# dominikh/jello

Hardware: AMD Instinct MI355X
Metric: Mpixels/sec fine-raster + paths/sec, 100k-path 4096^2 scene (higher is better)
Workload: dtype f32

## Files before the change

### jello_amd/csrc/kernels_flatten.hip

```cpp
#include <hip/hip_runtime.h>
__shared__ double fl_atan_tab[9];
#define JD_ATAN_TAB_LDS fl_atan_tab
#include "kcommon.h"
#define FF_INLINE __device__ __forceinline__
#include "flatten_fast.h"

using namespace jk;
using namespace jd;

namespace {

struct CubicParams { float th0, th1, chord_len, err; };
struct EulerParams { float th0, th1, k0, k1, ch; };
struct CubicPoints { V2 p0, p1, p2, p3; };
struct PointDeriv { V2 point, deriv; };
struct PathTagData { uint32_t tag_byte; MonoidK<5> monoid; };

#define DERIV_THRESH 1e-6f
#define DERIV_THRESH_SQUARED (DERIV_THRESH * DERIV_THRESH)
#define DERIV_EPS 1e-6f
#define SUBDIV_LIMIT (1.0f / 65536.0f)
#define K1_THRESH 1e-3f
#define DIST_THRESH 1e-3f
#define TANGENT_THRESH 1e-6f
// ... 725 lines not shown
            MonoidK<5> tot5;
            if (SCAN == 1) __syncthreads();
            const MonoidK<5> ex = block_excl_scan_monoid<5>(reduce_tag(tag_word), sh, &tot5);
            pm = monoid_add(prefix, ex);
            if (tag_monoids.ok(word_ix)) {
                store_tm(&tag_monoids.p[word_ix], pm);
            } else {
#pragma unroll
                for (int i = 0; i < 5; i++) pm.v[i] = 0u;
            }
            __syncthreads();
        } else {
            pm = load_tm(tag_monoids, word_ix);
        }
        const uint32_t ix0 = word_ix * 4u;
        for (uint32_t q = 0u; q < 12u; q++) {
            const uint32_t sl = ix0 * 3u + q;
            if (sl < cap) counts[sl] = 0u;
        }
        uint32_t th = 0u, tl = 0u;
#pragma unroll
        for (uint32_t k = 0; k < 4u; k++) {
            const uint32_t ix = ix0 + k;
            if (ix >= n_tags) continue;
            const MonoidK<5> tm = monoid_add(pm, reduce_tag(tag_word & ((1u << (k * 8u)) - 1u)));
            const uint32_t tag_byte = (tag_word >> (k * 8u)) & 0xffu;
            const uint32_t style_flags = scene.rd(cfg->layout.style_base + tm.v[3] - 2u);
            const bool is_stroke = (style_flags & JL_STYLE_FLAGS_STYLE) != 0u;
            const uint32_t path_ix = tm.v[4];
            if ((tag_byte & JL_PATH_TAG_PATH) != 0u && path_bboxes.ok(path_ix)) {
                path_bboxes.p[path_ix].draw_flags = ((style_flags & JL_STYLE_FLAGS_FILL) == 0u) ? 0u : 1u;
                path_bboxes.p[path_ix].trans_ix = tm.v[0] - 1u;
            }
            const uint32_t seg_type = tag_byte & JL_PATH_TAG_SEG_TYPE;
            const bool curved = seg_type != JL_PATH_TAG_LINETO;
            if (seg_type != 0u) {
                if (!is_stroke) {
                    if (curved) nh[blk][k] = 1u; else nl[blk][k] = 1u;
                } else if ((tag_byte & JL_PATH_TAG_SUBPATH_END) != 0u) {
                    if (curved) nl[blk][k] = 1u;
                } else {
                    if (curved) { nh[blk][k] = 2u; nl[blk][k] = 1u; } else { nl[blk][k] = 3u; }
                }
            }
            th += nh[blk][k];
            tl += nl[blk][k];
        }
        MonoidK<2> m, tot;
        m.v[0] = th; m.v[1] = tl;
        const MonoidK<2> e2 = block_excl_scan_monoid<2>(m, sh, &tot);
        eh[blk] = wg_h + e2.v[0];
        el[blk] = wg_l + e2.v[1];
        wg_h += tot.v[0];
        wg_l += tot.v[1];
        __syncthreads();
    }
    if (threadIdx.x == 0) {
        sh_base[0] = wg_h ? atomicAdd(&counters[0], wg_h) : 0u;
        sh_base[1] = wg_l ? atomicAdd(&counters[FL_CTR_LIGHT], wg_l) : 0u;
    }
    __syncthreads();
#pragma unroll
    for (uint32_t blk = 0; blk < PSC_BLOCKS; blk++) {
        const uint32_t ix0 = ((blockIdx.x * PSC_BLOCKS + blk) * JL_WG + threadIdx.x) * 4u;
        uint32_t ph = sh_base[0] + eh[blk], pl = sh_base[1] + el[blk];
#pragma unroll
        for (uint32_t k = 0; k < 4u; k++) {
            const uint32_t ix = ix0 + k;
            uint32_t sub = 0u;
            for (uint32_t q = 0; q < nh[blk][k]; q++, sub++, ph++)
                if (ph < cap) list[ph] = ix * 3u + sub;
            for (uint32_t q = 0; q < nl[blk][k]; q++, sub++, pl++)
                if (pl < cap) list[cap - 1u - pl] = ix * 3u + sub;
        }
    }
}

JD void run_item(const JlConfig* cfg, const Scene& s, Out& o, uint32_t slot, EulerJob& job, uint32_t& path_ix_out) {
    uint32_t ix = slot / 3u, sub = slot - ix * 3u;
    Seg g = load_seg(s, ix);
    uint32_t path_ix = g.tag.monoid.v[4];
    path_ix_out = path_ix;
    uint32_t style_ix = g.tag.monoid.v[3];
    uint32_t trans_ix = g.tag.monoid.v[0];
    uint32_t style_flags = g.style_flags;
    job.path_ix = path_ix; job.trans_ix = trans_ix;
    Xf transform;
    {
        uint32_t base = cfg->layout.transform_base + trans_ix * 6u;
        transform.m0 = u2f(s.scene.rd(base)); transform.m1 = u2f(s.scene.rd(base + 1u)); transform.m2 = u2f(s.scene.rd(base + 2u));
        transform.m3 = u2f(s.scene.rd(base + 3u)); transform.t0 = u2f(s.scene.rd(base + 4u)); transform.t1 = u2f(s.scene.rd(base + 5u));
    }
    CubicPoints pts = read_path_segment(s, g.tag, g.is_stroke);
    if (g.is_stroke) {
        float linewidth = u2f(s.scene.rd(cfg->layout.style_base + style_ix + 1u));
        float offset = 0.5f * linewidth;
        bool is_stroke_cap_marker = (g.tag.tag_byte & JL_PATH_TAG_SUBPATH_END) != 0u;
        if (is_stroke_cap_marker) {
            V2 tangent = cubic_start_tangent(pts.p0, pts.p1, pts.p2, pts.p3);
            V2 offset_tangent = offset * normalize(tangent);
            V2 n = v2(offset_tangent.y * -1.0f, offset_tangent.x * 1.0f);
            draw_cap(o, path_ix, (style_flags & JL_STYLE_FLAGS_START_CAP_MASK) >> 2, pts.p0, pts.p0 - n, pts.p0 + n, -offset_tangent, transform);
        } else {
            const float TT = TANGENT_THRESH * TANGENT_THRESH;
            V2 tan_prev = cubic_end_tangent(pts.p0, pts.p1, pts.p2, pts.p3);
            if (dot(tan_prev, tan_prev) < TT) tan_prev = v2(TANGENT_THRESH, 0.0f);
            V2 offset_tangent = offset * normalize(tan_prev);
            V2 n_prev = v2(offset_tangent.y * -1.0f, offset_tangent.x * 1.0f);
            if (sub < 2u) {
                V2 tan_start = cubic_start_tangent(pts.p0, pts.p1, pts.p2, pts.p3);
                if (dot(tan_start, tan_start) < TT) tan_start = v2(TANGENT_THRESH, 0.0f);
                V2 n_start = offset * normalize(v2(-tan_start.y, tan_start.x));
                job.valid = true; job.cubic = pts; job.local_to_device = transform;
                if (sub == 0u) { job.offset = offset; job.start_p = pts.p0 + n_start; job.end_p = pts.p3 + n_prev; }
                else { job.offset = -offset; job.start_p = pts.p0 - n_start; job.end_p = pts.p3 - n_prev; }
            } else {
                PathTagData ntag = compute_tag_monoid(s, ix + 1u);
                CubicPoints npts = read_path_segment(s, ntag, true);
                bool n_is_closed = (ntag.tag_byte & JL_PATH_TAG_SEG_TYPE) == JL_PATH_TAG_LINETO;
                bool n_is_marker = (ntag.tag_byte & JL_PATH_TAG_SUBPATH_END) != 0u;
                bool do_join = !n_is_marker || n_is_closed;
                if (do_join) {
                    V2 tan_next = cubic_start_tangent(npts.p0, npts.p1, npts.p2, npts.p3);
                    if (dot(tan_next, tan_next) < TT) tan_next = v2(TANGENT_THRESH, 0.0f);
                    V2 tnn = normalize(tan_next);
                    V2 n_next = v2((offset * tnn.y) * -1.0f, (offset * tnn.x) * 1.0f);
                    draw_join(o, path_ix, style_flags, pts.p3, tan_prev, tan_next, n_prev, n_next, transform);
                } else {
                    draw_cap(o, path_ix, (style_flags & JL_STYLE_FLAGS_END_CAP_MASK), pts.p3, pts.p3 + n_prev, pts.p3 - n_prev, offset_tangent, transform);
                }
            }
        }
    } else {
        job.valid = true; job.cubic = pts; job.local_to_device = transform;
        job.offset = 0.0f; job.start_p = pts.p0; job.end_p = pts.p3;
    }
}

#ifndef FLQ_STACK
#define FLQ_STACK 448u
#endif
#ifndef FLQ_LEAVES
#define FLQ_LEAVES 640u
#endif
#ifndef FLQ_MAX_LEVEL
#define FLQ_MAX_LEVEL 9u
#endif
struct FlBatch {
    uint32_t jhead[64];
    uint32_t stack[FLQ_STACK];
    uint32_t l_tpos[FLQ_LEAVES];
    uint16_t l_key[FLQ_LEAVES];
    uint16_t l_link[FLQ_LEAVES];
    uint32_t unsure[128];
    uint32_t n_stack, n_leaves, bail, n_unsure;
};

struct NodeResult {
    bool accept;
    CubicParams cp;
};
struct NodeEnds {
    V2 last_p, last_q;
    float last_t;
    V2 point, deriv;
    float t1;
};
JD NodeEnds node_ends(V2 p0, V2 p1, V2 p2, V2 p3, uint32_t level, uint32_t t0_u) {
    const float dt = u2f((127u - level) << 23);
    const float t0 = (float)t0_u * dt;
    NodeEnds r;
    if (t0_u == 0u) {
        r.last_p = p0;
        r.last_q = start_deriv(p0, p1, p2, p3);
        r.last_t = 0.0f;
    } else {
        PointDeriv pq0 = eval_cubic_and_deriv(p0, p1, p2, p3, t0);
        r.last_t = t0;
        if (dot(pq0.deriv, pq0.deriv) < DERIV_THRESH_SQUARED) {
            PointDeriv n0 = eval_cubic_and_deriv(p0, p1, p2, p3, t0 - DERIV_EPS);
            pq0.deriv = n0.deriv;
            pq0.point = n0.point;
            r.last_t = t0 - DERIV_EPS;
        }
        r.last_p = pq0.point;
        r.last_q = pq0.deriv;
    }
    const IntervalEnd ie = interval_end(p0, p1, p2, p3, t0 + dt);
    r.point = ie.pq.point;
    r.deriv = ie.pq.deriv;
    r.t1 = ie.t1;
    return r;
}
JD NodeResult node_test(V2 p0, V2 p1, V2 p2, V2 p3, float scale, uint32_t level, uint32_t t0_u) {
    const float tol = 0.25f;
    const float dt = u2f((127u - level) << 23);
    const NodeEnds ne = node_ends(p0, p1, p2, p3, level, t0_u);
    const float actual_dt = ne.t1 - ne.last_t;
    NodeResult r;
    r.cp = cubic_from_points_derivs(ne.last_p, ne.point, ne.last_q, ne.deriv, actual_dt);
    r.accept = r.cp.err * scale <= tol || dt <= SUBDIV_LIMIT;
    return r;
}
JD int node_test_fast(V2 p0, V2 p1, V2 p2, V2 p3, float scale, uint32_t level, uint32_t t0_u, float* v_est, float* delta) {
    const float tol = 0.25f;
    const NodeEnds ne = node_ends(p0, p1, p2, p3, level, t0_u);
    const float actual_dt = ne.t1 - ne.last_t;
    const V2 chord = ne.point - ne.last_p;
    const V2 q0 = ne.last_q, q1 = ne.deriv;
    *v_est = 0.0f; *delta = 0.0f;
    if (dot(chord, chord) < DERIV_THRESH_SQUARED) {
        const float chord_err = sqrt_((float)(9.0 / 32.0) * (dot(q0, q0) + dot(q1, q1))) * actual_dt;
        return (chord_err * scale <= tol) ? ffast::FF_ACCEPT : ffast::FF_REJECT;
    }
    return ffast::ff_decide_interval(chord.x, chord.y, q0.x, q0.y, q1.x, q1.y, actual_dt, scale, tol, v_est, delta);
}
JD CubicParams piece_angles(const NodeEnds& ne) {
    const V2 chord = ne.point - ne.last_p;
    const float chord_squared = dot(chord, chord);
    CubicParams r;
    r.err = 0.0f;
    if (chord_squared < DERIV_THRESH_SQUARED) {
        r.th0 = 0.0f; r.th1 = 0.0f; r.chord_len = DERIV_THRESH;
        return r;
    }
    const V2 q0 = ne.last_q, q1 = ne.deriv;
    const V2 h0 = v2(q0.x * chord.x + q0.y * chord.y, q0.y * chord.x - q0.x * chord.y);
    const V2 h1 = v2(q1.x * chord.x + q1.y * chord.y, q1.x * chord.y - q1.y * chord.x);
    r.th0 = atan2_(h0.y, h0.x);
    r.th1 = atan2_(h1.y, h1.x);
    r.chord_len = sqrt_(chord_squared);
    return r;
}


struct JobState { V2 p0, p1, p2, p3; float scale, offset; uint32_t slot, path_ix, trans_ix; V2 t_start, t_end; };
#define FL_JOB_CURVE(JB, E, J)                                                                                                      \
    JobState JB;                                                                                                                    \
    JB.p0 = v2(read_lane_var(E.p0.x, J), read_lane_var(E.p0.y, J)); JB.p1 = v2(read_lane_var(E.p1.x, J), read_lane_var(E.p1.y, J)); \
    JB.p2 = v2(read_lane_var(E.p2.x, J), read_lane_var(E.p2.y, J)); JB.p3 = v2(read_lane_var(E.p3.x, J), read_lane_var(E.p3.y, J)); \
    JB.scale = read_lane_var(E.scale, J)
#define FL_JOB_PIECE(JB, E, SLOT, J)                                                                                                \
    FL_JOB_CURVE(JB, E, J); JB.offset = read_lane_var(E.offset, J);                                                                 \
    JB.slot = read_lane_var(SLOT, J); JB.path_ix = read_lane_var(E.path_ix, J); JB.trans_ix = read_lane_var(E.trans_ix, J);         \
    JB.t_start = v2(read_lane_var(E.t_start.x, J), read_lane_var(E.t_start.y, J));                                                  \
    JB.t_end = v2(read_lane_var(E.t_end.x, J), read_lane_var(E.t_end.y, J))

#ifdef FL_FAST_CHECK
__device__ uint32_t g_ff_stats[8];
#endif
#ifndef FL_WAVES_PER_EU
#define FL_WAVES_PER_EU 4
#endif
#ifndef FL_BLOCKS_PER_CU
#define FL_BLOCKS_PER_CU 4
#endif
#ifdef FL_TIMING
#define FL_TL_WAVES 8192u
#define FL_TL_BATCHES 15u
#define FL_TL_WORDS (2u + 3u * FL_TL_BATCHES)
__device__ unsigned long long g_fl_timeline[FL_TL_WAVES * FL_TL_WORDS];
#endif
__global__ __launch_bounds__(JL_WG) __attribute__((amdgpu_waves_per_eu(FL_WAVES_PER_EU, FL_WAVES_PER_EU))) void k_flatten_items(const JlConfig* __restrict__ cfg, Buf<uint32_t> scene, Buf<JlTagMonoid> tag_monoids,
                                                         Buf<JlPathBbox> path_bboxes, const uint32_t* __restrict__ list,
                                                         uint32_t* __restrict__ counters, uint32_t cap, uint32_t* __restrict__ counts,
                                                         FlTemp T, uint32_t debug) {
    __shared__ FlBatch sh_batch[JL_WG / 64];
    Scene s;
    s.cfg = cfg; s.scene = scene; s.tag_monoids = tag_monoids;
    uint32_t n_heavy = umin_(counters[0], cap), n_light = umin_(counters[FL_CTR_LIGHT], cap - n_heavy);
    uint32_t n = n_heavy + n_light;
    const uint32_t units_h = n_heavy / 64u + (n_heavy % 64u != 0u ? 1u : 0u);
    const uint32_t units = units_h + n_light / 64u + (n_light % 64u != 0u ? 1u : 0u);
    const uint32_t n_groups = umin_(umax_(gridDim.x / FL_BLOCKS_PER_CU, 1u), FL_DEAL_GROUPS), group = blockIdx.x % n_groups;
    if (group >= units) return;
#ifdef FL_TIMING
    const unsigned long long tl_entry = wall_clock64();
    const uint32_t tl_wave = blockIdx.x * (JL_WG / 64u) + (threadIdx.x >> 6);
    uint32_t tl_n = 0u;
#endif
    atan_tab_fill();
    __syncthreads();
    const uint32_t lane = lane_id();
    FlBatch& B = sh_batch[threadIdx.x >> 6];
    Out o;
    o.cfg = cfg; o.T = T; o.home_s = o.home_r = blockIdx.x % T.K; o.failed_s = o.failed_r = false; o.slot = 0u;
    if ((debug & 1u) != 0u) o.home_s = o.home_r = 0u;
#ifdef FL_SOAK_HOME0
    o.home_s = o.home_r = 0u;
#endif
    o.cursor = 0u; o.a_first = 0u; o.a_spos = 0u; o.a_rpos = 0u;
    for (;;) {
        uint32_t k = 0u;
        if (lane == 0u) k = atomicAdd(&counters[FL_CTR_DEAL + FL_DEAL_STRIDE * group], 1u);
        k = uni(k);
        const uint32_t u = k * n_groups + group;
        if (u >= units) break;
        const bool heavy = u < units_h;
        const uint32_t t_first = heavy ? u * 64u : n_heavy + (u - units_h) * 64u;
        const uint32_t t_end = umin_(t_first + 64u, heavy ? n_heavy : n);
        const uint32_t t = t_first + lane;
#ifdef FL_TIMING
        const unsigned long long tl_start = wall_clock64() | (heavy ? 1ull << 63 : 0ull);
        uint32_t tl_info = 0u;
#define FL_TL_END()                                                                                      \
    do {                                                                                                 \
        if (lane == 0u && tl_wave < FL_TL_WAVES && tl_n < FL_TL_BATCHES) {                               \
            g_fl_timeline[tl_wave * FL_TL_WORDS + 2u + 3u * tl_n] = tl_start;                            \
            g_fl_timeline[tl_wave * FL_TL_WORDS + 3u + 3u * tl_n] = wall_clock64();                      \
            g_fl_timeline[tl_wave * FL_TL_WORDS + 4u + 3u * tl_n] = tl_info;                             \
        }                                                                                                \
        tl_n++;                                                                                          \
    } while (0)
#else
#define FL_TL_END() do {} while (0)
#endif
        if (__builtin_amdgcn_ballot_w64(o.failed_s) != 0ull) { o.home_s = fl_next_home(T, o.home_s, 0); o.failed_s = false; }
        if (__builtin_amdgcn_ballot_w64(o.failed_r) != 0ull) { o.home_r = fl_next_home(T, o.home_r, 1); o.failed_r = false; }
        EulerJob job;
        job.valid = false; job.path_ix = 0u; job.trans_ix = 0u; job.offset = 0.0f;
        job.start_p = v2(0, 0); job.end_p = v2(0, 0);
        job.cubic.p0 = job.cubic.p1 = job.cubic.p2 = job.cubic.p3 = v2(0, 0);
        job.local_to_device = xf_identity();
        uint32_t slot = FL_INVALID;
        if (t < t_end) {
            slot = heavy ? list[t] : list[cap - 1u - (t - n_heavy)];
            o.slot = slot; o.cursor = 0u; o.a_first = 0u; o.a_spos = 0u; o.a_rpos = 0u;
            uint32_t path_ix;
            run_item(cfg, s, o, slot, job, path_ix);
            if (!job.valid) counts[slot] = o.cursor;
        }
        EulerLane e;
        euler_begin(e, job);
        const bool active = job.valid && !e.done;
        if (__builtin_amdgcn_ballot_w64(active) == 0ull) {
            FL_TL_END();
            continue;
        }
        B.jhead[lane] = 0u;
        {
            const uint64_t am = __builtin_amdgcn_ballot_w64(active);
            if (active) B.stack[(uint32_t)__builtin_popcountll(am & ((1ull << lane) - 1ull))] = lane;
            if (lane == 0u) { B.n_stack = (uint32_t)__builtin_popcountll(am); B.n_leaves = 0u; B.bail = 0u; B.n_unsure = 0u; }
        }
        wave_sync();
#ifdef FL_SPLIT_NO_A
        if (lane == 0u) B.n_stack = 0u;
        wave_sync();
#endif
        for (;;) {
#ifdef FL_TIMING
            tl_info += 1u << 16;
#endif
            const uint32_t ns = uni(B.n_stack);
            const uint32_t nu = (uint32_t)__builtin_amdgcn_readfirstlane((int)B.n_unsure);
            if (ns == 0u && nu == 0u) break;
            const bool exact_round = ns == 0u || nu >= 64u;
            const uint32_t take = umin_(exact_round ? nu : ns, 64u);
            const bool has = lane < take;
            const uint32_t node = has ? (exact_round ? B.unsure[nu - 1u - lane] : B.stack[ns - 1u - lane]) : 0u;
            wave_sync();
            const uint32_t j = node & 63u, level = (node >> 6) & 31u, t0_u = node >> 11;
            FL_JOB_CURVE(jb, e, j);
            int kind = ffast::FF_UNSURE;
            if (exact_round) {
                if (has) kind = node_test(jb.p0, jb.p1, jb.p2, jb.p3, jb.scale, level, t0_u).accept ? ffast::FF_ACCEPT : ffast::FF_REJECT;
            } else if (has) {
                float v_est, delta;
                kind = node_test_fast(jb.p0, jb.p1, jb.p2, jb.p3, jb.scale, level, t0_u, &v_est, &delta);
#ifdef FL_FAST_CHECK
            }
            if (!exact_round) {
                bool c_unsure = false, c_contra = false, c_viol = false;
                if (has) {
                    float v2_, d2_;
                    const int k2 = node_test_fast(jb.p0, jb.p1, jb.p2, jb.p3, jb.scale, level, t0_u, &v2_, &d2_);
                    const NodeResult rx = node_test(jb.p0, jb.p1, jb.p2, jb.p3, jb.scale, level, t0_u);
                    const float vx = rx.cp.err * jb.scale;
                    c_unsure = k2 == ffast::FF_UNSURE;
                    c_contra = (k2 == ffast::FF_ACCEPT && !rx.accept) || (k2 == ffast::FF_REJECT && rx.accept);
                    c_viol = (d2_ > 0.0f && !(abs_(v2_ - vx) <= d2_)) || (d2_ == 0.0f && k2 != ffast::FF_UNSURE && v2_ != 0.0f);
                }
                const uint32_t n0 = (uint32_t)__builtin_popcountll(__builtin_amdgcn_ballot_w64(has));
                const uint32_t n1 = (uint32_t)__builtin_popcountll(__builtin_amdgcn_ballot_w64(c_unsure));
                const uint32_t n2 = (uint32_t)__builtin_popcountll(__builtin_amdgcn_ballot_w64(c_contra));
                const uint32_t n3 = (uint32_t)__builtin_popcountll(__builtin_amdgcn_ballot_w64(c_viol));
                if (lane == 0u) {
                    atomicAdd(&g_ff_stats[0], n0);
                    if (n1) atomicAdd(&g_ff_stats[1], n1);
                    if (n2) atomicAdd(&g_ff_stats[2], n2);
                    if (n3) atomicAdd(&g_ff_stats[3], n3);
                }
#endif
            }
            const bool acc = has && kind == ffast::FF_ACCEPT, rej = has && kind == ffast::FF_REJECT, uns = has && kind == ffast::FF_UNSURE;
            const uint64_t accm = __builtin_amdgcn_ballot_w64(acc), rejm = __builtin_amdgcn_ballot_w64(rej), unsm = __builtin_amdgcn_ballot_w64(uns);
            const uint32_t n_acc = (uint32_t)__builtin_popcountll(accm), n_rej = (uint32_t)__builtin_popcountll(rejm);
            const uint32_t n_uns = (uint32_t)__builtin_popcountll(unsm);
            const uint32_t nl = uni(B.n_leaves);
            const uint32_t ns_left = exact_round ? ns : ns - take, nu_left = exact_round ? nu - take : nu;
            const bool too_deep = __builtin_amdgcn_ballot_w64(rej && level + 1u > FLQ_MAX_LEVEL) != 0ull;
            if (too_deep || ns_left + 2u * n_rej > FLQ_STACK || nl + n_acc > FLQ_LEAVES) {
                if (lane == 0u) B.bail = 1u;
                wave_sync();
                break;
            }
            const uint64_t below = (1ull << lane) - 1ull;
            if (rej) {
                const uint32_t pos = ns_left + 2u * (uint32_t)__builtin_popcountll(rejm & below);
                B.stack[pos] = j | ((level + 1u) << 6) | ((2u * t0_u + 1u) << 11);
                B.stack[pos + 1u] = j | ((level + 1u) << 6) | ((2u * t0_u) << 11);
            }
            if (acc) {
                const uint32_t li = nl + (uint32_t)__builtin_popcountll(accm & below);
                B.l_tpos[li] = node;
                B.l_key[li] = (uint16_t)((t0_u << (FLQ_MAX_LEVEL - level)) << 7);
                const uint32_t prev = atomicExch(&B.jhead[j], li + 1u);
                B.l_link[li] = (uint16_t)((j << 10) | prev);
            }
            if (uns) B.unsure[nu_left + (uint32_t)__builtin_popcountll(unsm & below)] = node;
            if (lane == 0u) { B.n_stack = ns_left + 2u * n_rej; B.n_leaves = nl + n_acc; B.n_unsure = nu_left + n_uns; }
            wave_sync();
        }
        const bool bail = uni(B.bail) != 0u;
        const uint32_t nl = bail ? 0u : uni(B.n_leaves);
#ifdef FL_TIMING
        tl_info = (tl_info & 0x7fff0000u) | (nl & 0xffffu) | (bail ? 1u << 31 : 0u);
#endif
        uint32_t rec_base = 0u;
        if (nl != 0u && lane == 0u) rec_base = fl_grab<1>(T, o.home_r, nl, o.failed_r);
        rec_base = (uint32_t)__builtin_amdgcn_readlane((int)rec_base, 0);
#ifdef FL_SPLIT_NO_B
        for (uint32_t lbase = nl; lbase < nl; lbase += 64u) {
#else
        for (uint32_t lbase = 0u; lbase < nl; lbase += 64u) {
#endif
            const uint32_t li = lbase + lane;
            const bool has = li < nl;
            const uint32_t node = has ? B.l_tpos[li] : 0u;
            const uint32_t j = node & 63u, level = (node >> 6) & 31u, t0_u = node >> 11;
            FL_JOB_PIECE(jb, e, slot, j);
            if (has) {
                const NodeEnds ne = node_ends(jb.p0, jb.p1, jb.p2, jb.p3, level, t0_u);
                const CubicParams cp = piece_angles(ne);
                const PieceParams pp = piece_params(cp, jb.scale, jb.offset);
                const uint32_t fl = piece_flags(pp.robust, ne.t1, jb.offset, t0_u == 0u);
                const uint32_t r = rec_base + li;
                if (rec_base != FL_INVALID)
                    piece_record_write(T.recs + (size_t)r * 4u, ne.last_p, ne.point, pp.ep.th0, pp.ep.th1, pp.int0, pp.integral, pp.noff, jb.slot,
                                       jb.path_ix, jb.trans_ix, fl, 0u, jb.t_start, jb.t_end);
                B.l_key[li] = (uint16_t)(B.l_key[li] | pp.n_u);
            }
        }
        wave_sync();
        if (nl != 0u) {
            uint32_t total = 0u;
            if (active)
                for (uint32_t q = B.jhead[lane]; q != 0u; q = B.l_link[q - 1u] & 1023u) total += B.l_key[q - 1u] & 127u;
            if (active) counts[slot] = total;
            const uint32_t incl = wave_incl_scan_u32(total);
            const uint32_t batch_total = (uint32_t)__builtin_amdgcn_readlane((int)incl, 63);
            const bool together = batch_total <= ((debug & 4u) != 0u ? 48u : FL_MAX_GRAB);
            uint32_t grab = 0u;
            if (together) {
                if (lane == 0u) grab = fl_grab<0>(T, o.home_s, batch_total, o.failed_s);
            } else if (active && total != 0u) {
                grab = fl_grab<0>(T, o.home_s, total, o.failed_s);
            }
            for (uint32_t li = lane; li < nl; li += 64u) {
                const uint32_t j = B.l_link[li] >> 10, key = B.l_key[li];
                uint32_t first = 0u;
                for (uint32_t q = B.jhead[j]; q != 0u; q = B.l_link[q - 1u] & 1023u) {
                    const uint32_t k2 = B.l_key[q - 1u];
                    if ((k2 >> 7) < (key >> 7)) first += k2 & 127u;
                }
                B.l_tpos[li] = first;
            }
            {
                const uint32_t base0 = (uint32_t)__builtin_amdgcn_readlane((int)grab, 0);
                B.unsure[lane] = together ? (base0 == FL_INVALID ? FL_INVALID : base0 + (incl - total)) : grab;
            }
            wave_sync();
            for (uint32_t li = lane; li < nl; li += 64u) {
                const uint32_t j = B.l_link[li] >> 10, key = B.l_key[li], first = B.l_tpos[li];
                const uint32_t r = rec_base + li, jb = B.unsure[j];
                if (rec_base != FL_INVALID && (key >> 7) != 0u) piece_record_set_first(T.recs + (size_t)r * 4u, first);
                if (jb == FL_INVALID) continue;
                if (rec_base != FL_INVALID) piece_slots_write(T.sinfo, jb + first, key & 127u, r);
                else for (uint32_t i = 0u; i < (key & 127u); i++) T.sinfo[jb + first + i] = make_uint2(0u, 0u);
            }
            wave_sync();
        }
        if (__builtin_expect(bail, 0)) {
            o.slot = slot; o.cursor = 0u; o.a_first = 0u; o.a_spos = 0u; o.a_rpos = 0u;
            bool have = active;
            auto finish = [&]() -> bool {
                if (e.done && have) {
                    counts[o.slot] = o.cursor;
                    have = false;
                }
                return __builtin_amdgcn_ballot_w64(!e.done) != 0ull;
            };
            flatten_euler_wave(o, e, finish);
        }
        FL_TL_END();
    }
#ifdef FL_TIMING
    if (lane == 0u && tl_wave < FL_TL_WAVES) {
        g_fl_timeline[tl_wave * FL_TL_WORDS] = tl_entry;
        g_fl_timeline[tl_wave * FL_TL_WORDS + 1u] = tl_n;
    }
#endif
#undef FL_TL_END
#undef FL_JOB_PIECE
#undef FL_JOB_CURVE
}

#ifndef FL_LINES_WAVES_PER_EU
#define FL_LINES_WAVES_PER_EU 4
#endif
__global__ __launch_bounds__(JL_WG) __attribute__((amdgpu_waves_per_eu(FL_LINES_WAVES_PER_EU, FL_LINES_WAVES_PER_EU))) void k_flatten_lines(const JlConfig* __restrict__ cfg, Buf<uint32_t> scene, const uint32_t* __restrict__ counters,
                                                         FlTemp T, const uint32_t* __restrict__ bases, uint32_t n_slots, Buf<JlLineSoup> lines) {
    atan_tab_fill();
    const uint32_t lines_lim = umin_(cfg->lines_size, lines.n);
    const uint2* __restrict__ sinfo = T.sinfo;
    const uint4* __restrict__ recs = T.recs;
    const uint32_t n_r = T.K * T.R;
    uint32_t ru[FL_MAX_REGIONS], used[FL_MAX_REGIONS];
    uint32_t units = 0u;
#pragma unroll
    for (uint32_t c = 0u; c < FL_MAX_REGIONS; c++) {
        ru[c] = units;
        used[c] = c < T.K ? umin_(*fl_cursor_in(counters, c, 0), T.R) : 0u;
        units += (used[c] + JL_WG - 1u) / JL_WG;
    }
    auto fetch_info = [&](uint32_t u) -> uint2 {
        if (u >= units) return make_uint2(0u, 0u);
        uint32_t c = 0u, first_unit = 0u, in_use = used[0];
#pragma unroll
        for (uint32_t q = 1u; q < FL_MAX_REGIONS; q++)
            if (u >= ru[q] && used[q] != 0u) { c = q; first_unit = ru[q]; in_use = used[q]; }
        const uint32_t in_region = (u - first_unit) * JL_WG + threadIdx.x;
        return in_region < in_use ? sinfo[(size_t)c * T.R + in_region] : make_uint2(0u, 0u);
    };
    auto state_of = [&](uint2 si) -> uint32_t {
        if (si.x >= n_r) return 0u;
        return (si.y & FL_INFO_PIECE) != 0u ? 2u : ((si.y & FL_INFO_DIRECT) != 0u ? 1u : 0u);
    };
    auto fetch_rec = [&](uint32_t state, uint32_t r, uint4& r0, uint4& r1, uint4& r2, uint4& r3) {
        r0 = r1 = r2 = r3 = make_uint4(0u, 0u, 0u, 0u);
        const uint4* rec = recs + (size_t)r * 4u;
        if (state != 0u) { r0 = rec[0]; r1 = rec[1]; }
        if (state == 2u) { r2 = rec[2]; r3 = rec[3]; }
    };
    const uint32_t G = gridDim.x;
    uint2 si_a = fetch_info(blockIdx.x), si_b = fetch_info(blockIdx.x + G);
    uint32_t st_a = state_of(si_a);
    uint4 a0, a1, a2, a3;
    fetch_rec(st_a, si_a.x, a0, a1, a2, a3);
    for (uint32_t u = blockIdx.x; u < units; u += G) {
        const uint32_t st = st_a;
        const uint2 si = si_a;
        const uint4 r0 = a0, r1 = a1, r2 = a2, r3 = a3;
        si_a = si_b;
        st_a = state_of(si_a);
        fetch_rec(st_a, si_a.x, a0, a1, a2, a3);
        si_b = fetch_info(u + 2u * G);
        uint32_t widx[3] = {0xffffffffu, 0xffffffffu, 0xffffffffu};
        uint2 wdat[3] = {make_uint2(0u, 0u), make_uint2(0u, 0u), make_uint2(0u, 0u)};
        if (st == 1u) {
            const uint32_t item = DREC_ITEM(r), k = DREC_K(r);
            if (item < n_slots) {
                const uint32_t dst = bases[item] + k;
                if (dst < lines_lim) {
                    widx[0] = dst * 3u; wdat[0] = make_uint2(DREC_PATH_IX(r), 0u);
                    widx[1] = dst * 3u + 1u; wdat[1] = DREC_P0(r);
                    widx[2] = dst * 3u + 2u; wdat[2] = DREC_P1(r);
                }
            }
        } else if (st == 2u) {
            const uint32_t n_u = SINFO_LINES(si), i = SINFO_LINE(si);
            const uint32_t flags = PREC_FLAGS(r);
            const bool last_of_item = i + 1u == n_u && (flags & FL_PC_ENDS_AT_ONE) != 0u;
            const uint32_t slot = PREC_ITEM(r), k = PREC_FIRST_LINE(r) + i;
            Xf tr;
            if ((flags & FL_PC_NO_OFFSET) != 0u) {
                tr = xf_identity();
            } else {
                uint32_t tb = cfg->layout.transform_base + PREC_TRANS_IX(r) * 6u;
                tr.m0 = u2f(scene.rd(tb)); tr.m1 = u2f(scene.rd(tb + 1u)); tr.m2 = u2f(scene.rd(tb + 2u));
                tr.m3 = u2f(scene.rd(tb + 3u)); tr.t0 = u2f(scene.rd(tb + 4u)); tr.t1 = u2f(scene.rd(tb + 5u));
            }
            const uint32_t slot_base = slot < n_slots ? bases[slot] : 0u;
            V2 lp1;
            if (last_of_item) {
                lp1 = PREC_T_END(r);
#if defined(FL_LSPLIT) && FL_LSPLIT == 1
            } else if (true) {
                lp1 = v2(PREC_ES_P0(r).x + (float)i, PREC_ES_P1(r).y + PREC_TH0(r) + PREC_TH1(r) + PREC_INT0(r) + PREC_INTEGRAL(r) + PREC_NOFF(r));
#endif
            } else {
                const EulerParams ep = es_params_from_angles(PREC_TH0(r), PREC_TH1(r));
                const float noff = PREC_NOFF(r), n = (float)n_u;
                const float tt = (float)(i + 1u) / n;
                float sarg = tt;
                const uint32_t robust = flags & FL_PC_ROBUST;
                if (robust != FL_ROBUST_LOW_K1) {
                    const PieceAB ab = piece_ab(ep, noff, robust);
                    const float int0 = PREC_INT0(r), integral = PREC_INTEGRAL(r);
                    float uu = integral * tt + int0;
                    float inv;
                    if (robust == FL_ROBUST_LOW_DIST) inv = pow23_abs_(uu) * sign_(uu); else inv = espc_int_inv_approx(uu);
                    sarg = (inv - ab.b) / ab.a;
                }
                lp1 = es_seg_eval_with_offset(PREC_ES_P0(r), PREC_ES_P1(r), ep, sarg, noff);
            }
            const V2 q = xf_apply(tr, lp1);
            if (slot < n_slots) {
                const uint32_t dst = slot_base + k;
                const bool fwd = (flags & FL_PC_FORWARD) != 0u;
                const bool has_next = !last_of_item && dst + 1u < lines_lim;
                const uint2 hdr = make_uint2(PREC_PATH_IX(r), 0u), pt = make_uint2(f2u(q.x), f2u(q.y));
                if (dst < lines_lim) {
                    if (k == 0u) {
                        uint2* w = (uint2*)lines.p;
                        const V2 qs = xf_apply(tr, PREC_T_START(r));
                        w[(size_t)dst * 3u] = hdr;
                        w[(size_t)dst * 3u + (fwd ? 1u : 2u)] = make_uint2(f2u(qs.x), f2u(qs.y));
                    }
                    widx[0] = dst * 3u + (fwd ? 2u : 1u); wdat[0] = pt;
                    if (has_next) {
                        widx[1] = dst * 3u + 3u; wdat[1] = hdr;
                        widx[2] = dst * 3u + (fwd ? 4u : 5u); wdat[2] = pt;
                    }
                }
            }
        }
        {
            uint2* w = (uint2*)lines.p;
#pragma unroll
            for (int j = 0; j < 3; j++)
#if defined(FL_LSPLIT) && FL_LSPLIT == 2
                if (widx[j] == 0xfffffffeu) w[widx[j]] = wdat[j];
#else
                if (widx[j] != 0xffffffffu) w[widx[j]] = wdat[j];
#endif
        }
    }
}

JD uint32_t fkey(float f) { uint32_t b = f2u(f); return (b & 0x80000000u) ? ~b : (b | 0x80000000u); }
JD float fkey_inv(uint32_t k) { return u2f((k & 0x80000000u) ? (k & 0x7fffffffu) : ~k); }

JD bool fb_tag_has_extent(const uint32_t* __restrict__ bases, uint32_t n_tags, const JlLineSoup* lines, uint32_t total, uint32_t pos) {
    uint32_t g = 0u, ge = n_tags;
    while (ge - g > 1u) {
        const uint32_t mid = g + (ge - g) / 2u;
        if (umin_(bases[3u * mid], total) <= pos) g = mid; else ge = mid;
    }
    const uint32_t lo = umin_(bases[3u * g], total);
    const uint32_t hi = (g + 1u < n_tags) ? umin_(bases[3u * g + 3u], total) : total;
    float bx0 = 1e31f, by0 = 1e31f, bx1 = -1e31f, by1 = -1e31f;
    for (uint32_t i = lo; i < hi; i++) {
        const JlLineSoup l = lines[i];
        bx0 = fmin_(bx0, fmin_(l.p0[0], l.p1[0])); by0 = fmin_(by0, fmin_(l.p0[1], l.p1[1]));
        bx1 = fmax_(bx1, fmax_(l.p0[0], l.p1[0])); by1 = fmax_(by1, fmax_(l.p0[1], l.p1[1]));
    }
    return bx1 > bx0 || by1 > by0;
}

JD void fb_merge(Buf<JlPathBbox> path_bboxes, uint32_t path_ix, int32_t x0, int32_t y0, int32_t x1, int32_t y1, bool atomic) {
    if (!path_bboxes.ok(path_ix)) return;
    if (x0 == 0x7fffffff && y0 == 0x7fffffff && x1 == (int32_t)0x80000000 && y1 == (int32_t)0x80000000) return;
    JlPathBbox* out = &path_bboxes.p[path_ix];
    if (!atomic) {
        out->x0 = imin_(out->x0, x0); out->y0 = imin_(out->y0, y0);
        out->x1 = imax_(out->x1, x1); out->y1 = imax_(out->y1, y1);
    } else {
        const int32_t cx0 = __hip_atomic_load(&out->x0, __ATOMIC_RELAXED, __HIP_MEMORY_SCOPE_AGENT);
        const int32_t cy0 = __hip_atomic_load(&out->y0, __ATOMIC_RELAXED, __HIP_MEMORY_SCOPE_AGENT);
        const int32_t cx1 = __hip_atomic_load(&out->x1, __ATOMIC_RELAXED, __HIP_MEMORY_SCOPE_AGENT);
        const int32_t cy1 = __hip_atomic_load(&out->y1, __ATOMIC_RELAXED, __HIP_MEMORY_SCOPE_AGENT);
        if (x0 < cx0) atomicMin(&out->x0, x0);
        if (y0 < cy0) atomicMin(&out->y0, y0);
        if (x1 > cx1) atomicMax(&out->x1, x1);
        if (y1 > cy1) atomicMax(&out->y1, y1);
    }
}

#define FB_NONE 0xffffffffu
#ifndef FB_TARGET_WAVES
#define FB_TARGET_WAVES 2048u
#endif
__global__ __launch_bounds__(JL_WG) void k_flatten_bbox(const JlConfig* __restrict__ cfg, const JlBump* __restrict__ bump,
                                                        const uint32_t* __restrict__ bases, uint32_t n_slots, Buf<JlLineSoup> lines,
                                                        Buf<JlPathBbox> path_bboxes, uint32_t* __restrict__ zero, uint32_t zero_n) {
    for (uint32_t i = blockIdx.x * JL_WG + threadIdx.x; i < zero_n; i += gridDim.x * JL_WG) zero[i] = 0u;
    const uint32_t n_tags = n_slots / 3u;
    const uint32_t total = umin_(umin_(bump->lines, cfg->lines_size), lines.n);
    const uint32_t lane = lane_id();
    const uint32_t n_waves = (gridDim.x * JL_WG) >> 6;
    const uint32_t batches = umin_(umax_(((total + 63u) / 64u) / FB_TARGET_WAVES, 1u), 8u);
    for (uint64_t start64 = (uint64_t)((blockIdx.x * JL_WG + threadIdx.x) >> 6) * batches * 64u; start64 < total;
         start64 += (uint64_t)n_waves * batches * 64u) {
        const uint32_t start = (uint32_t)start64;
        const uint32_t end = (uint32_t)(start64 + (uint64_t)batches * 64u < total ? start64 + (uint64_t)batches * 64u : total);
        uint32_t p_before = FB_NONE;
        if (start > 0u) p_before = lines.p[start - 1u].path_ix;
        bool skip_before = false;
        uint32_t p_shared = FB_NONE;
        uint32_t c_path = FB_NONE;
        int32_t cx0 = 0x7fffffff, cy0 = 0x7fffffff, cx1 = (int32_t)0x80000000, cy1 = (int32_t)0x80000000;
        JlLineSoup l_next = {};
        if (start + lane < total) l_next = lines.p[start + lane];
        for (uint32_t base = start; base < total; base += 64u) {
            const bool ext = base >= end;
            if (ext && c_path == FB_NONE) break;
            const uint32_t pos = base + lane;
            const JlLineSoup l = l_next;
            if (!ext && pos + 64u < total) l_next = lines.p[pos + 64u];
            bool valid = pos < (ext ? total : end);
// ... 167 lines not shown
```

Measured before the change: 21070.

## Deduplicate identical adjacent Euler jobs in wave subdivision, replicating leaves to followers

Before subdivision, each lane compares its cubic control points and scale with the previous lane. Lanes whose job is identical to their neighbour's become followers and are left off the subdivision stack. When a leader's segment is accepted, the leaf is replicated for the run of followers using a wave inclusive scan for leaf offsets. This removes redundant subdivision work for duplicate segments, such as repeated stroke or instance geometry, at the cost of extra cross-lane shuffles, a scan per round and a serial per-lane loop.

```diff
diff --git a/jello_amd/csrc/kernels_flatten.hip b/jello_amd/csrc/kernels_flatten.hip
--- a/jello_amd/csrc/kernels_flatten.hip
+++ b/jello_amd/csrc/kernels_flatten.hip
@@ -1051,13 +1051,13 @@
         const uint32_t t = t_first + lane;
 #ifdef FL_TIMING
         const unsigned long long tl_start = wall_clock64() | (heavy ? 1ull << 63 : 0ull);
-        uint32_t tl_info = 0u;
+        uint32_t tl_info = 0u, tl_jobs = 0u;
 #define FL_TL_END()                                                                                      \
     do {                                                                                                 \
         if (lane == 0u && tl_wave < FL_TL_WAVES && tl_n < FL_TL_BATCHES) {                               \
             g_fl_timeline[tl_wave * FL_TL_WORDS + 2u + 3u * tl_n] = tl_start;                            \
             g_fl_timeline[tl_wave * FL_TL_WORDS + 3u + 3u * tl_n] = wall_clock64();                      \
-            g_fl_timeline[tl_wave * FL_TL_WORDS + 4u + 3u * tl_n] = tl_info;                             \
+            g_fl_timeline[tl_wave * FL_TL_WORDS + 4u + 3u * tl_n] = tl_info | (unsigned long long)tl_jobs << 32; \
         }                                                                                                \
         tl_n++;                                                                                          \
     } while (0)
@@ -1087,10 +1087,22 @@
             continue;
         }
         B.jhead[lane] = 0u;
+        uint64_t followers = 0ull;
         {
+            uint32_t diff = (f2u(e.p0.x) ^ lane_prev(f2u(e.p0.x), 0u)) | (f2u(e.p0.y) ^ lane_prev(f2u(e.p0.y), 0u));
+            diff |= (f2u(e.p1.x) ^ lane_prev(f2u(e.p1.x), 0u)) | (f2u(e.p1.y) ^ lane_prev(f2u(e.p1.y), 0u));
+            diff |= (f2u(e.p2.x) ^ lane_prev(f2u(e.p2.x), 0u)) | (f2u(e.p2.y) ^ lane_prev(f2u(e.p2.y), 0u));
+            diff |= (f2u(e.p3.x) ^ lane_prev(f2u(e.p3.x), 0u)) | (f2u(e.p3.y) ^ lane_prev(f2u(e.p3.y), 0u));
+            diff |= f2u(e.scale) ^ lane_prev(f2u(e.scale), 0u);
             const uint64_t am = __builtin_amdgcn_ballot_w64(active);
-            if (active) B.stack[(uint32_t)__builtin_popcountll(am & ((1ull << lane) - 1ull))] = lane;
-            if (lane == 0u) { B.n_stack = (uint32_t)__builtin_popcountll(am); B.n_leaves = 0u; B.bail = 0u; B.n_unsure = 0u; }
+            const uint64_t same = __builtin_amdgcn_ballot_w64(diff == 0u) & am & (am << 1);
+            if ((debug & 16u) == 0u) followers = same;
+#ifdef FL_TIMING
+            tl_jobs = (uint32_t)__builtin_popcountll(am) | (uint32_t)__builtin_popcountll(followers) << 8;
+#endif
+            const uint64_t lm = am & ~followers;
+            if (((lm >> lane) & 1ull) != 0ull) B.stack[(uint32_t)__builtin_popcountll(lm & ((1ull << lane) - 1ull))] = lane;
+            if (lane == 0u) { B.n_stack = (uint32_t)__builtin_popcountll(lm); B.n_leaves = 0u; B.bail = 0u; B.n_unsure = 0u; }
         }
         wave_sync();
 #ifdef FL_SPLIT_NO_A
@@ -1143,9 +1155,11 @@
 #endif
             }
             const bool acc = has && kind == ffast::FF_ACCEPT, rej = has && kind == ffast::FF_REJECT, uns = has && kind == ffast::FF_UNSURE;
-            const uint64_t accm = __builtin_amdgcn_ballot_w64(acc), rejm = __builtin_amdgcn_ballot_w64(rej), unsm = __builtin_amdgcn_ballot_w64(uns);
-            const uint32_t n_acc = (uint32_t)__builtin_popcountll(accm), n_rej = (uint32_t)__builtin_popcountll(rejm);
-            const uint32_t n_uns = (uint32_t)__builtin_popcountll(unsm);
+            const uint64_t rejm = __builtin_amdgcn_ballot_w64(rej), unsm = __builtin_amdgcn_ballot_w64(uns);
+            const uint32_t n_rej = (uint32_t)__builtin_popcountll(rejm), n_uns = (uint32_t)__builtin_popcountll(unsm);
+            const uint32_t run = acc ? 1u + (uint32_t)__builtin_ctzll(~((followers >> j) >> 1)) : 0u;
+            const uint32_t acc_incl = wave_incl_scan_u32(run);
+            const uint32_t n_acc = (uint32_t)__builtin_amdgcn_readlane((int)acc_incl, 63);
             const uint32_t nl = uni(B.n_leaves);
             const uint32_t ns_left = exact_round ? ns : ns - take, nu_left = exact_round ? nu - take : nu;
             const bool too_deep = __builtin_amdgcn_ballot_w64(rej && level + 1u > FLQ_MAX_LEVEL) != 0ull;
@@ -1161,11 +1175,14 @@
                 B.stack[pos + 1u] = j | ((level + 1u) << 6) | ((2u * t0_u) << 11);
             }
             if (acc) {
-                const uint32_t li = nl + (uint32_t)__builtin_popcountll(accm & below);
-                B.l_tpos[li] = node;
-                B.l_key[li] = (uint16_t)((t0_u << (FLQ_MAX_LEVEL - level)) << 7);
-                const uint32_t prev = atomicExch(&B.jhead[j], li + 1u);
-                B.l_link[li] = (uint16_t)((j << 10) | prev);
+                const uint32_t li0 = nl + acc_incl - run;
+                for (uint32_t q = 0u; q < run; q++) {
+                    const uint32_t li = li0 + q;
+                    B.l_tpos[li] = node + q;
+                    B.l_key[li] = (uint16_t)((t0_u << (FLQ_MAX_LEVEL - level)) << 7);
+                    const uint32_t prev = atomicExch(&B.jhead[j + q], li + 1u);
+                    B.l_link[li] = (uint16_t)(((j + q) << 10) | prev);
+                }
             }
             if (uns) B.unsure[nu_left + (uint32_t)__builtin_popcountll(unsm & below)] = node;
             if (lane == 0u) { B.n_stack = ns_left + 2u * n_rej; B.n_leaves = nl + n_acc; B.n_unsure = nu_left + n_uns; }
```

New measurement: 21270, median of 6. No clear change (+0.9%).
